# yoyololicon/pytorch-NMF

Hardware: AMD Instinct MI355X
Metric: MU GFLOP/s (algorithmic 8*N*C*R per iteration), dense NMF 4096x65536 rank-128 beta=1; MU iterations/s alongside (higher is better)
Workload: dtype f16; 1 GPU; NMF 4096x65536 rank=128 beta=1 (BASELINE configs[1]); preset=cfg1, rows=4096, cols_per_gpu=65536, rank=128, precision=f16, parallelism=single GPU, nsplit_h=16, nsplit_w=1, block_rows_h=256, block_rows_w=256, launch=eager launches

## Files before the change

include/nmfmu.h:

```cpp
#ifndef NMFMU_H_
#define NMFMU_H_

#include <stddef.h>
#include <stdint.h>

#ifdef __cplusplus
extern "C" {
#endif

#define NMFMU_ABI_VERSION 10

#define NMFMU_OK 0
#define NMFMU_ERR_UNSUPPORTED (-2)
#define NMFMU_ERR_ARG (-3)
#define NMFMU_ERR_ALLOC (-4)

#define NMFMU_PREC_BF16 0
#define NMFMU_PREC_BF16X3 1
#define NMFMU_PREC_F16 2
#define NMFMU_PREC_F16X 3
#define NMFMU_PREC_F16R 4

#define NMFMU_BETA_KL 0
#define NMFMU_BETA_EUC 1
#define NMFMU_BETA_IS 2
#define NMFMU_BETA_GEN 3

#define NMFMU_STAGE_REG 0
#define NMFMU_STAGE_DMA 1
#define NMFMU_STAGE_DMA_NOP2 3
#define NMFMU_STAGE_DMA_LDSTR 4
#define NMFMU_STAGE_DMA_SPLIT 2

typedef struct nmfmu_factor {
  float* f;
  void* p1_hi;
  void* p1_lo;
  void* p2_hi;
  void* p2_lo;
  float* colsum;
  float* colsum_part;
  int32_t rows;
  int32_t rows_pad;
} nmfmu_factor;

typedef struct nmfmu_step {
  const void* xp;
  nmfmu_factor owner;
  nmfmu_factor panel;
  float* slab_num;
  float* slab_den;
  int32_t rank;
  int32_t r_pad;
  int32_t nsplit;
  int32_t precision;
  int32_t stage;
  int32_t block_rows;
  float beta;
  float gamma;
  float l1, l2;
  uint32_t* status;
  void* stamps;
} nmfmu_step;

int nmfmu_abi_version(void);
int nmfmu_abi_check(int compiled_against);
int nmfmu_pad_rows(int rows);
int nmfmu_pad_rank(int rank);
int nmfmu_beta_kind(float beta);
int nmfmu_supported(int r_pad, int precision);
int nmfmu_block_rows(int r_pad, int precision, float beta);
int nmfmu_choose_nsplit(int owner_rows_pad, int panel_rows_pad, int block_rows, int num_cu);
#define NMFMU_KERNEL_FUSED 0
#define NMFMU_KERNEL_PP 1
#define NMFMU_KERNEL_SP 2
int nmfmu_kernel_family(int r_pad, int precision, float beta);
int nmfmu_pp_lds_transpose_supported(int r_pad, int precision, float beta);
int nmfmu_choose_nsplit_for(int owner_rows_pad, int panel_rows_pad, int r_pad, int precision, float beta, int block_rows, int num_cu);
int nmfmu_step_block_rows(int owner_rows_pad, int panel_rows_pad, int r_pad, int precision, float beta, int num_cu);
size_t nmfmu_xp_bytes(int owner_rows_pad, int panel_rows_pad, int precision);
size_t nmfmu_image_bytes(int rows_pad, int r_pad);
size_t nmfmu_slab_bytes(int owner_rows_pad, int r_pad, int nsplit);
size_t nmfmu_colsum_part_bytes(int rows_pad, int r_pad);

// ... 314 lines not shown
```

pytorch-nmf_amd/csrc/nmfmu_capi.hip:

```cpp
#include <hip/hip_runtime.h>
#include <stdint.h>

#include <algorithm>
#include <cstdlib>
#include <new>
#include <vector>

#include "../../include/nmfmu.h"
#include "nmfmu_aux.h"
#include "nmfmu_fused.h"
#include "nmfmu_pp.h"
#include "nmfmu_sp.h"
#include "nmfmu_sp2.h"

#ifndef NMFMU_SP
#define NMFMU_SP 1
#endif
#ifndef NMFMU_SP2
#define NMFMU_SP2 1
#endif
#ifndef NMFMU_FUSE_APPLY_TWO_ACC
#define NMFMU_FUSE_APPLY_TWO_ACC 1
#endif

using namespace nmfmu;

namespace {

inline hipStream_t S(void* s) { return reinterpret_cast<hipStream_t>(s); }
inline bool is_f16(int precision) {
  return precision == NMFMU_PREC_F16 || precision == NMFMU_PREC_F16X || precision == NMFMU_PREC_F16R;
}
inline bool x_is_f32(int precision) { return precision == NMFMU_PREC_BF16X3 || precision == NMFMU_PREC_F16X; }

#ifdef NMFMU_DEBUG_HOOKS
static int env_int(const char* name, int dflt) {
  const char* v = std::getenv(name);
  return v && *v ? std::atoi(v) : dflt;
}
static void* g_pp_debug = nullptr;
#endif
#ifndef NMFMU_PP_F16R
#define NMFMU_PP_F16R 1
#endif
static bool pp_eligible(int r_pad, int precision, float beta) {
  return nmfmu_beta_kind(beta) == NMFMU_BETA_KL && r_pad <= 128 &&
         (precision == NMFMU_PREC_F16 || precision == NMFMU_PREC_BF16 || (NMFMU_PP_F16R && precision == NMFMU_PREC_F16R));
}
static bool pp_ldstr_eligible(int r_pad, int precision, float beta) {
  return pp_eligible(r_pad, precision, beta) && pp_trl_available(r_pad, is_f16(precision) ? kOpF16 : kOpBf16, kModeMU);
}
static bool sp_eligible(int r_pad, int precision, float beta) {
  return NMFMU_SP && nmfmu_beta_kind(beta) == NMFMU_BETA_KL && r_pad == 256 && precision == NMFMU_PREC_F16;
}
static bool sp2_eligible(int r_pad, int precision, float beta) {
  const int k = nmfmu_beta_kind(beta);
  return NMFMU_SP2 && (k == NMFMU_BETA_IS || k == NMFMU_BETA_GEN) && r_pad == 128 && precision == NMFMU_PREC_F16;
}
static int kernel_beta_kind(float beta) {
  if (beta == 0.5f) return kSqrt;
  if (beta == 1.5f) return kSqrt3;
  return nmfmu_beta_kind(beta);
}

struct GramRef {
  const float* gram;
  const void* hi;
  const void* lo;
  const float* scale;
};

int fused_dispatch(const nmfmu_step* st, int mode, float* loss_part, int M, int K, hipStream_t s,
                   const float* fuse_kl_den = nullptr, bool fuse_apply = false, const GramRef* gm = nullptr) {
  if (!st || !st->owner.p1_hi || !st->panel.p1_hi) return NMFMU_ERR_ARG;
  if (!st->xp && (mode == kModeMU || mode == kModeXB)) return NMFMU_ERR_ARG;
  if (st->owner.rows_pad % kRowPad || st->panel.rows_pad % kRowPad) return NMFMU_ERR_ARG;
  if (st->block_rows != 128 && st->block_rows != 256) return NMFMU_ERR_ARG;
  if (st->stage != NMFMU_STAGE_DMA && st->stage != NMFMU_STAGE_DMA_SPLIT && st->stage != NMFMU_STAGE_DMA_NOP2 &&
      st->stage != NMFMU_STAGE_DMA_LDSTR)
    return NMFMU_ERR_UNSUPPORTED;
  const bool ldstr = st->stage == NMFMU_STAGE_DMA_LDSTR && mode != kModeLoss;
  if (ldstr && (mode != kModeMU || st->block_rows != 256 || !pp_ldstr_eligible(st->r_pad, st->precision, st->beta)))
    return NMFMU_ERR_UNSUPPORTED;
  if (st->stage == NMFMU_STAGE_DMA_SPLIT && mode == kModeMU && !(st->precision == NMFMU_PREC_BF16X3)) {
    if (nmfmu_beta_kind(st->beta) != NMFMU_BETA_KL || st->block_rows != 128) return NMFMU_ERR_UNSUPPORTED;
    mode = kModeMU2;
  }
  if (st->r_pad != pad_rank(st->rank) || st->nsplit < 1) return NMFMU_ERR_ARG;
  const bool x3 = st->precision == NMFMU_PREC_BF16X3;
  if (x3 && (!st->owner.p1_lo || !st->panel.p1_lo)) return NMFMU_ERR_ARG;
  const int kind = nmfmu_beta_kind(st->beta);
  if (st->precision == NMFMU_PREC_F16R && kind == NMFMU_BETA_EUC) return NMFMU_ERR_UNSUPPORTED;
  FusedArgs a{};
  a.xp = st->xp;
  a.p1_hi = static_cast<const uint16_t*>(st->panel.p1_hi);
  a.p1_lo = static_cast<const uint16_t*>(st->panel.p1_lo);
  a.p2_hi = static_cast<const uint16_t*>(st->panel.p2_hi);
  a.p2_lo = static_cast<const uint16_t*>(st->panel.p2_lo);
  a.a1_hi = static_cast<const uint16_t*>(st->owner.p1_hi);
  a.a1_lo = static_cast<const uint16_t*>(st->owner.p1_lo);
  a.slab_num = st->slab_num;
  a.slab_den = st->slab_den;
  a.loss_part = loss_part;
  a.M = M;
  a.K = K;
  a.M_pad = st->owner.rows_pad;
  a.ktiles = st->panel.rows_pad / kBK;
  a.nsplit = st->nsplit;
  a.tiles_per_split = (a.ktiles + st->nsplit - 1) / st->nsplit;
  a.beta = st->beta;
  a.status = st->status;
  a.cs_owner = st->owner.colsum;
  a.cs_panel = st->panel.colsum;
  if (fuse_apply) {
    a.fuse_apply = 1;
    a.rank = st->rank;
    a.f = st->owner.f;
    a.kl_den = fuse_kl_den;
    a.o1_hi = static_cast<uint16_t*>(st->owner.p1_hi), a.o1_lo = static_cast<uint16_t*>(st->owner.p1_lo);
    a.o2_hi = static_cast<uint16_t*>(st->owner.p2_hi), a.o2_lo = static_cast<uint16_t*>(st->owner.p2_lo);
    a.colsum_part = st->owner.colsum_part;
    a.l1 = st->l1, a.l2 = st->l2, a.gamma = st->gamma;
  }
  if (mode == kModeMU2) {
    if (!a.slab_num || !a.p2_hi || fuse_apply) return NMFMU_ERR_ARG;
  } else if (mode == kModeXB) {
    if (kind != kEuc || x3 || st->block_rows != 128) return NMFMU_ERR_UNSUPPORTED;
    if (!a.p2_hi || (!fuse_apply && !a.slab_num)) return NMFMU_ERR_ARG;
    if (fuse_apply && (!gm || st->r_pad > 128)) return NMFMU_ERR_ARG;
    if (gm) {
      if (!gm->hi || !gm->lo || !gm->scale || (!fuse_apply && !a.slab_den)) return NMFMU_ERR_ARG;
      a.gram_hi = static_cast<const uint16_t*>(gm->hi), a.gram_lo = static_cast<const uint16_t*>(gm->lo);
      a.gram_scale = gm->scale;
    } else {
      a.slab_den = nullptr;
    }
  } else if (mode == kModeMU || mode == kModeDen) {
    if (!a.slab_num || !a.p2_hi || (x3 && !a.p2_lo)) return NMFMU_ERR_ARG;
    if (mode == kModeMU && kind != kKL && !a.slab_den) return NMFMU_ERR_ARG;
    if (mode == kModeDen && (kind != kGen || st->block_rows != 128)) return NMFMU_ERR_UNSUPPORTED;
  } else if (!loss_part) {
    return NMFMU_ERR_ARG;
  }
  const int grid = (st->owner.rows_pad / st->block_rows) * st->nsplit;
  if (st->block_rows == 256) {
    if (!st->xp || mode == kModeDen || !pp_eligible(st->r_pad, st->precision, st->beta)) return NMFMU_ERR_UNSUPPORTED;
    a.tiles_per_split = (a.tiles_per_split + 1) & ~1;
    a.debug = mode == kModeMU ? st->stamps : nullptr;
#ifdef NMFMU_DEBUG_HOOKS
    if (mode == kModeMU && g_pp_debug) a.debug = g_pp_debug;
#endif
    if (ldstr) a.o2_hi = nullptr;
    return launch_pp(st->r_pad, is_f16(st->precision) ? kOpF16 : kOpBf16, mode, a, grid, s, st->precision == NMFMU_PREC_F16R,
                      mode == kModeMU && loss_part != nullptr, ldstr);
  }
  if (mode == kModeMU && sp_eligible(st->r_pad, st->precision, st->beta)) {
    a.tiles_per_split = (a.tiles_per_split + 3) & ~3;
    a.debug = st->stamps;
#ifdef NMFMU_DEBUG_HOOKS
    if (g_pp_debug) a.debug = g_pp_debug;
#endif
    if (st->stage == NMFMU_STAGE_DMA_NOP2) a.o2_hi = nullptr;
    return launch_sp(st->r_pad, kOpF16, a, grid, s);
  }
  if (mode == kModeMU && sp2_eligible(st->r_pad, st->precision, st->beta)) {
    a.tiles_per_split = (a.tiles_per_split + 3) & ~3;
    return launch_sp2(st->r_pad, kernel_beta_kind(st->beta), a, grid, s);
  }
  const int kk = kernel_beta_kind(st->beta);
#ifdef NMFMU_DEBUG_HOOKS
  a.debug = mode == kModeXB ? g_pp_debug : nullptr;
#endif
  switch (st->r_pad) {
    case 32: return launch_fused_r32(kk, st->precision, mode, a, grid, s);
    case 64: return launch_fused_r64(kk, st->precision, mode, a, grid, s);
    case 128: return launch_fused_r128(kk, st->precision, mode, a, grid, s);
    case 256: return launch_fused_r256(kk, st->precision, mode, a, grid, s);
  }
  return NMFMU_ERR_UNSUPPORTED;
}

struct Timer {
  std::vector<hipEvent_t> ev;
};

}

extern "C" {

int nmfmu_abi_version(void) { return NMFMU_ABI_VERSION; }
int nmfmu_abi_check(int compiled_against) { return compiled_against == NMFMU_ABI_VERSION ? NMFMU_OK : NMFMU_ERR_ARG; }
int nmfmu_pad_rows(int rows) { return rows <= 0 ? NMFMU_ERR_ARG : pad_rows(rows); }
int nmfmu_pad_rank(int rank) {
  const int r = pad_rank(rank);
  return r < 0 ? NMFMU_ERR_UNSUPPORTED : r;
}
int nmfmu_beta_kind(float beta) {
  if (beta == 1.f) return NMFMU_BETA_KL;
  if (beta == 2.f) return NMFMU_BETA_EUC;
  if (beta == 0.f) return NMFMU_BETA_IS;
  return NMFMU_BETA_GEN;
}
int nmfmu_supported(int r_pad, int precision) {
  if (r_pad != 32 && r_pad != 64 && r_pad != 128 && r_pad != 256) return 0;
  if (precision == NMFMU_PREC_BF16) return 1;
// ... 127 lines not shown
                                      st->owner.colsum, S(stream))
             : nmfmu_mu_apply(st, nullptr, nullptr, 0, kl ? kl_den : nullptr, stream);
  }
  return e;
}

int nmfmu_colsum_nparts(const nmfmu_step* st) {
  if (!st || (st->block_rows != 128 && st->block_rows != 256)) return NMFMU_ERR_ARG;
  return st->nsplit == 1 ? st->owner.rows_pad / st->block_rows : st->owner.rows_pad / apply_stripe_rows(st->owner.rows_pad);
}

int nmfmu_pack_nparts(int rows_pad) { return rows_pad <= 0 ? NMFMU_ERR_ARG : rows_pad / apply_stripe_rows(rows_pad); }

int nmfmu_colsum_finalize(const nmfmu_factor* fac, int nparts, int r_pad, void* stream) {
  if (!fac || !fac->colsum || !fac->colsum_part || nparts <= 0) return NMFMU_ERR_ARG;
  return launch_colsum_finalize(fac->colsum_part, nparts, r_pad, fac->colsum, S(stream));
}

int nmfmu_slab_reduce(const nmfmu_step* st, float* num_out, float* den_out, void* stream) {
  if (!st || !num_out || !st->slab_num) return NMFMU_ERR_ARG;
  const int64_t plane = (int64_t)st->owner.rows_pad * st->r_pad;
  int e = launch_slab_reduce(st->slab_num, st->nsplit, plane, num_out, S(stream));
  if (e) return e;
  if (den_out) {
    if (!st->slab_den) return NMFMU_ERR_ARG;
    e = launch_slab_reduce(st->slab_den, st->nsplit, plane, den_out, S(stream));
  }
  return e;
}

static int apply_common(const nmfmu_step* st, const float* num, const float* den, int nslab, const float* kl_den,
                        int trainer, float ortho, float* grad, void* stream, int den_nslab = 0, int skip_colsum = 0) {
  if (!st || !st->owner.f) return NMFMU_ERR_ARG;
  const bool kl = nmfmu_beta_kind(st->beta) == NMFMU_BETA_KL;
  ApplyArgs a{};
  a.f = st->owner.f;
  a.num = num ? num : st->slab_num;
  a.den = num ? den : st->slab_den;
  a.nslab = num ? nslab : st->nsplit;
  a.kl_den = kl ? kl_den : nullptr;
  if (!a.num || a.nslab < 1) return NMFMU_ERR_ARG;
  a.den_nslab = den_nslab;
  a.skip_colsum = skip_colsum;
  if (kl ? !a.kl_den : !a.den) return NMFMU_ERR_ARG;
  a.p1_hi = st->owner.p1_hi, a.p1_lo = st->owner.p1_lo, a.p2_hi = st->owner.p2_hi, a.p2_lo = st->owner.p2_lo;
  a.colsum_part = st->owner.colsum_part, a.colsum = st->owner.colsum;
  a.rows = st->owner.rows, a.rank = st->rank, a.rows_pad = st->owner.rows_pad;
  a.l1 = st->l1, a.l2 = st->l2, a.gamma = st->gamma;
  a.trainer = trainer, a.ortho = ortho, a.grad = grad;
  a.f16 = is_f16(st->precision);
  a.status = st->status;
  if (!a.p1_hi || !a.p2_hi || !a.colsum || !a.colsum_part) return NMFMU_ERR_ARG;
  if (st->stage == NMFMU_STAGE_DMA_NOP2 && sp_eligible(st->r_pad, st->precision, st->beta)) a.p2_hi = a.p2_lo = nullptr;
  if (st->stage == NMFMU_STAGE_DMA_LDSTR) {
    if (st->block_rows != 256 || !pp_ldstr_eligible(st->r_pad, st->precision, st->beta)) return NMFMU_ERR_UNSUPPORTED;
    a.p2_hi = a.p2_lo = nullptr;
  }
  return launch_apply(st->r_pad, a, st->precision == NMFMU_PREC_BF16X3, false, S(stream));
}

int nmfmu_mu_apply(const nmfmu_step* st, const float* num, const float* den, int nslab, const float* kl_den,
                   void* stream) {
  return apply_common(st, num, den, nslab, kl_den, 0, 0.f, nullptr, stream);
}

int nmfmu_trainer_apply(const nmfmu_step* st, const float* num, const float* den, int nslab, const float* kl_den,
                        float ortho, float* grad, void* stream) {
  if (!(ortho >= 0.f)) return NMFMU_ERR_ARG;
  return apply_common(st, num, den, nslab, kl_den, 1, ortho, grad, stream);
}

int nmfmu_xb_supported(int r_pad, int precision, float beta) {
  if (nmfmu_beta_kind(beta) != NMFMU_BETA_EUC) return 0;
  if (r_pad != 32 && r_pad != 64 && r_pad != 128 && r_pad != 256) return 0;
  if (precision == NMFMU_PREC_F16X) return r_pad <= 128;
  return precision == NMFMU_PREC_BF16 || precision == NMFMU_PREC_F16;
}

int nmfmu_xb_partial(const nmfmu_step* st, void* stream) {
  if (!st) return NMFMU_ERR_ARG;
  if (!nmfmu_xb_supported(st->r_pad, st->precision, st->beta)) return NMFMU_ERR_UNSUPPORTED;
  return fused_dispatch(st, kModeXB, nullptr, st->owner.rows, st->panel.rows, S(stream));
}

int nmfmu_xb_step(const nmfmu_step* st, const void* g_hi, const void* g_lo, const float* g_scale, int phase, void* stream) {
  if (!st || !g_hi || !g_lo || !g_scale || phase < 0 || phase > 2) return NMFMU_ERR_ARG;
  if (!nmfmu_xb_supported(st->r_pad, st->precision, st->beta)) return NMFMU_ERR_UNSUPPORTED;
  const bool fuse = st->nsplit == 1 && st->owner.f && st->owner.p2_hi && st->owner.colsum && st->owner.colsum_part &&
                    st->r_pad <= 128;
  if (!fuse && !st->slab_den) return NMFMU_ERR_ARG;
  const GramRef gm{nullptr, g_hi, g_lo, g_scale};
  int e = 0;
  if (phase != 2) {
    e = fused_dispatch(st, kModeXB, nullptr, st->owner.rows, st->panel.rows, S(stream), nullptr, fuse, &gm);
    if (e) return e;
  }
  if (phase != 1 && !fuse)
    e = apply_common(st, nullptr, nullptr, 0, nullptr, 0, 0.f, nullptr, stream, 1, 1);
  return e;
}

int nmfmu_mu_step_allreduce(const nmfmu_step* st, nmfmu_comm* comm, float* xbuf, void* stream) {
  if (!st || !comm || !xbuf) return NMFMU_ERR_ARG;
  const bool kl = nmfmu_beta_kind(st->beta) == NMFMU_BETA_KL;
  const size_t plane = (size_t)st->owner.rows_pad * st->r_pad;
  const size_t tail = kl ? (size_t)st->r_pad : plane;
  if (kl && !st->panel.colsum) return NMFMU_ERR_ARG;
// ... 228 lines not shown
```

pytorch-nmf_amd/torchnmf_amd/_capi.py:

```python
from __future__ import annotations

import ctypes as C
import os
from typing import Optional

LIB_NAME = 'libnmfmu.so'
LIB_PATH = os.environ.get('NMFMU_LIB') or os.path.join(os.path.dirname(os.path.abspath(__file__)), LIB_NAME)

OK = 0
ERR_UNSUPPORTED = -2
ERR_ARG = -3
ERR_ALLOC = -4
PREC_BF16, PREC_BF16X3, PREC_F16, PREC_F16X, PREC_F16R = 0, 1, 2, 3, 4
STAGE_REG, STAGE_DMA, STAGE_DMA_SPLIT = 0, 1, 2
STAGE_DMA_NOP2 = 3
STAGE_DMA_LDSTR = 4
BETA_KL, BETA_EUC, BETA_IS, BETA_GEN = 0, 1, 2, 3
KERNEL_FUSED, KERNEL_PP, KERNEL_SP = 0, 1, 2

PRECISIONS = {'bf16': PREC_BF16, 'bf16x3': PREC_BF16X3, 'f16': PREC_F16, 'f16x': PREC_F16X, 'f16r': PREC_F16R}


class NmfmuError(RuntimeError):
    pass


class Factor(C.Structure):
    _fields_ = [('f', C.c_void_p), ('p1_hi', C.c_void_p), ('p1_lo', C.c_void_p), ('p2_hi', C.c_void_p),
                ('p2_lo', C.c_void_p), ('colsum', C.c_void_p), ('colsum_part', C.c_void_p), ('rows', C.c_int32),
                ('rows_pad', C.c_int32)]


class Step(C.Structure):
    _fields_ = [('xp', C.c_void_p), ('owner', Factor), ('panel', Factor), ('slab_num', C.c_void_p),
                ('slab_den', C.c_void_p), ('rank', C.c_int32), ('r_pad', C.c_int32), ('nsplit', C.c_int32),
                ('precision', C.c_int32), ('stage', C.c_int32), ('block_rows', C.c_int32), ('beta', C.c_float), ('gamma', C.c_float),
                ('l1', C.c_float), ('l2', C.c_float), ('status', C.c_void_p), ('stamps', C.c_void_p)]


class GemmDesc(C.Structure):
    _fields_ = [('a_hi', C.c_void_p), ('a_lo', C.c_void_p), ('b_hi', C.c_void_p), ('b_lo', C.c_void_p),
                ('m_pad', C.c_int32), ('n_pad', C.c_int32), ('k_pad', C.c_int32), ('precision', C.c_int32),
                ('beta', C.c_float), ('x', C.c_void_p), ('gn_hi', C.c_void_p), ('gn_lo', C.c_void_p),
                ('gp_hi', C.c_void_p), ('gp_lo', C.c_void_p), ('out', C.c_void_p), ('m_valid', C.c_int32),
                ('n_valid', C.c_int32), ('ops', C.c_int32), ('t_batch', C.c_int32), ('t_rank', C.c_int32),
                ('t_taps', C.c_int32), ('t_lh', C.c_int32), ('tile_rows', C.c_int32), ('n_ld', C.c_int32), ('k_len', C.c_int32), ('k_split', C.c_int32),
                ('tail_rows', C.c_int32), ('rag_c0', C.c_int32), ('rag_channels', C.c_int32),
                ('win_nd', C.c_int32), ('win_lh', C.c_int32 * 3), ('win_taps', C.c_int32 * 3), ('win_channels', C.c_int32),
                ('win_pitch', C.c_int32), ('win_fold', C.c_int32), ('t_koff', C.c_void_p), ('stage_mode', C.c_int32)]


ABI_VERSION = 10
EPI_RATIO, EPI_F32, EPI_LOSS, EPI_FOLD = 0, 1, 2, 3
OPS_PLANES, OPS_B_HU, OPS_B_HUT, OPS_A_HU, OPS_A_WIN = 0, 1, 2, 3, 4

SIGNATURES = {
    'nmfmu_abi_version': (C.c_int, []),
    'nmfmu_abi_check': (C.c_int, [C.c_int]),
    'nmfmu_pad_rows': (C.c_int, [C.c_int]),
    'nmfmu_pad_rank': (C.c_int, [C.c_int]),
    'nmfmu_beta_kind': (C.c_int, [C.c_float]),
    'nmfmu_supported': (C.c_int, [C.c_int, C.c_int]),
    'nmfmu_block_rows': (C.c_int, [C.c_int, C.c_int, C.c_float]),
    'nmfmu_step_block_rows': (C.c_int, [C.c_int, C.c_int, C.c_int, C.c_int, C.c_float, C.c_int]),
    'nmfmu_choose_nsplit': (C.c_int, [C.c_int, C.c_int, C.c_int, C.c_int]),
    'nmfmu_kernel_family': (C.c_int, [C.c_int, C.c_int, C.c_float]),
    'nmfmu_pp_lds_transpose_supported': (C.c_int, [C.c_int, C.c_int, C.c_float]),
    'nmfmu_choose_nsplit_for': (C.c_int, [C.c_int, C.c_int, C.c_int, C.c_int, C.c_float, C.c_int, C.c_int]),
    'nmfmu_xp_bytes': (C.c_size_t, [C.c_int, C.c_int, C.c_int]),
# ... 238 lines not shown
```

pytorch-nmf_amd/torchnmf_amd/engine.py:

```python
from __future__ import annotations

import ctypes as C
import os
from typing import Optional

import torch

from . import _capi


def _ptr(t: Optional[torch.Tensor]) -> Optional[int]:
    return None if t is None else t.data_ptr()


class HipBackend:

    name = 'hip'

    def __init__(self):
        self.lib = _capi.load()
        if not torch.cuda.is_available():
            raise _capi.NmfmuError('torchnmf_amd needs a ROCm device (MI355X); none is visible and there is no '
                                   'CPU fallback')

# ... 389 lines not shown
            return None
        in_range, exact = cls.f16_stats(V, W, H, be) if dims_ok else (False, False)
        level = 2 if (in_range and exact) else (1 if in_range else 0)
        if level == 1 and not (hasattr(_capi, 'PREC_F16X') and be.supported(r_pad, _capi.PREC_F16X)
                               and os.environ.get('TORCHNMF_AMD_AUTO_F16X', '1') != '0'):
            level = 0
        if group is not None:
            import torch.distributed as dist
            flag = torch.tensor([level], dtype=torch.int32, device=V.device)
            dist.all_reduce(flag, op=dist.ReduceOp.MIN, group=group)
            level = int(flag.item())
            if level == 1 and not (hasattr(_capi, 'PREC_F16X') and be.supported(r_pad, _capi.PREC_F16X)):
                level = 0
        return {2: 'f16', 1: 'f16x', 0: None}[level]

    @classmethod
    def auto_mode(cls, V, W, H, r_pad, be, beta, group=None) -> Optional[str]:
        mode = cls.auto_single_plane(V, W, H, r_pad, be, group)
        if (mode == 'f16x' and float(beta) != 2.0 and hasattr(_capi, 'PREC_F16R') and be.supported(r_pad, _capi.PREC_F16R)
                and os.environ.get('TORCHNMF_AMD_AUTO_F16R', '1') != '0'):
            mode = 'f16r'
        return mode

    def __init__(self, V, W, H, beta, l1=0.0, l2=0.0, precision='auto', stage=None, group=None, backend=None,
                 update_W=True, update_H=True, block_rows=None, allow_f16=False, ar_overlap=None, allow_gram=False,
                 ar_direct=None):
        self.be = backend if backend is not None else DEFAULT_BACKEND_FACTORY()
        self.group = group
        self.beta = float(beta)
        self.kl = self.beta == 1.0
        N, Cc = V.shape
        R = W.shape[1]
        assert W.shape == (Cc, R) and H.shape == (N, R)
        if V.stride(1) != 1 or V.dtype != torch.float32:
            V = V.float().contiguous()
        self.rank = R
        self.r_pad = self.be.pad_rank(R)
        if precision in (None, 'auto'):
            precision = self.auto_mode(V, W, H, self.r_pad, self.be, self.beta, group) if allow_f16 else None
            if precision is None:
                if not self.be.supported(self.r_pad, _capi.PREC_BF16X3):
                    raise NotImplementedError(
                        f"precision='auto' found no mode for rank {R} that meets the 1e-4 parity bar on the fused kernels "
                        f"(fp16 operands -- 'f16', or 'f16x' with an fp32 target -- need both dimensions >= {self.F16_MIN_DIM} "
                        f"and data within fp16's range; split bf16 stops at rank 128); pass precision='bf16' (factors "
                        f"~1e-3), 'f16' or 'f16x' explicitly")
                precision = 'bf16x3'
        if precision not in _capi.PRECISIONS:
            raise ValueError(f"precision must be one of {sorted(_capi.PRECISIONS)} or 'auto', got {precision!r}")
        self.precision_name = precision
        self.precision = _capi.PRECISIONS[precision]
        if not self.be.supported(self.r_pad, self.precision):
            raise NotImplementedError(f'precision {precision!r} is not available for rank {R} (padded {self.r_pad})')
        if stage is None:
            nop2 = (hasattr(self.be, 'kernel_family') and hasattr(_capi, 'STAGE_DMA_NOP2') and float(beta) == 1.0
                    and self.r_pad == 256 and self.be.kernel_family(self.r_pad, self.precision, float(beta)) == _capi.KERNEL_SP
                    and os.environ.get('TORCHNMF_AMD_NO_P2', '1') != '0')
            stage = _capi.STAGE_DMA_NOP2 if nop2 else _capi.STAGE_DMA
            if (group is None and update_W and block_rows in (None, 256) and hasattr(self.be, 'pp_lds_transpose_supported')
                    and self.be.pp_lds_transpose_supported(self.r_pad, self.precision, float(beta))
                    and self.be.block_rows(self.r_pad, self.precision, float(beta)) == 256):
                stage = _capi.STAGE_DMA_LDSTR
        self.gram_path = (allow_gram and self.beta == 2.0 and group is None and block_rows in (None, 128)
                          and hasattr(self.be, 'xb_supported') and self.be.xb_supported(self.r_pad, self.precision, self.beta)
                          and os.environ.get('TORCHNMF_AMD_BETA2_GRAM', '1') != '0')
        gamma = mu_gamma(self.beta)
        dev = V.device

        self.fW = FactorBuf(W, self.r_pad, self.precision, self.be)
        self.fH = FactorBuf(H, self.r_pad, self.precision, self.be)
        self.flags = torch.tensor([0, 0x7f800000], dtype=torch.int32, device=dev)
        self.status = torch.zeros(1, dtype=torch.int32, device=dev)
        n_pad, c_pad = self.fH.rows_pad, self.fW.rows_pad
        def tile_rows(m_pad, k_pad):
            if block_rows is not None:
                return block_rows
            if hasattr(self.be, 'step_block_rows'):
                return self.be.step_block_rows(m_pad, k_pad, self.r_pad, self.precision, self.beta, dev)
            return self.be.block_rows(self.r_pad, self.precision, self.beta)
        br = tile_rows(n_pad, c_pad)
        self.block_rows = br
        xp_h = self.be.pack_x(V, False, self.precision, br, n_pad, c_pad, self.flags)
        ns_h = self._nsplit(n_pad, c_pad, br, dev)
        need_den = False if self.kl else ('one' if self.gram_path else True)
        self.step_h = StepBuf(xp_h, self.fH, self.fW, R, self.r_pad, ns_h, self.precision, stage, br, self.beta, gamma,
                              l1, l2, need_den=need_den, status=self.status)
        self.step_w = None
        if update_W:
            brw = tile_rows(c_pad, n_pad)
            xp_w = self.be.pack_x(V, True, self.precision, brw, c_pad, n_pad, None)
            ns_w = self._nsplit(c_pad, n_pad, brw, dev)
            self.step_w = StepBuf(xp_w, self.fW, self.fH, R, self.r_pad, ns_w, self.precision, stage, brw, self.beta,
                                  gamma, l1, l2, need_den=need_den, status=self.status)
        self.gm = self.be.gram_alloc(self.r_pad, dev) if self.gram_path else None
        self.timer: Optional[KernelTimer] = None
        self.refresh_images()
        self.loss_part = torch.empty(max((n_pad // br) * ns_h, 1), dtype=torch.float32, device=dev)
        self.loss_out = torch.zeros(1, dtype=torch.float64, device=dev)
        self._riding = None
        self._riding_pending = False
        if (group is None and self.kl and self.step_w is not None and update_H and hasattr(self.be, 'riding_supported')
                and os.environ.get('TORCHNMF_AMD_RIDING_LOSS', '1') != '0' and V.dtype == torch.float32 and V.stride(1) == 1
                and self.be.riding_supported(self.step_w)):
            self._riding = {'V': V, 'bufs': None}
        if group is not None:
            tail = self.r_pad if self.kl else self.step_h.plane
            self.xbuf = torch.empty(self.step_h.plane + tail, dtype=torch.float32, device=dev)
            explicit_direct = bool(ar_direct)
            if ar_direct is None:
                ar_direct = os.environ.get('TORCHNMF_AMD_COMM', 'torch') == 'c'
            self._comm = None
            if ar_direct and hasattr(self.be, 'comm_init'):
                self._comm = self.be.comm_init(group, dev)
                ar_overlap = False
            elif explicit_direct:
                raise _capi.NmfmuError("allreduce='direct' needs the library's own RCCL communicator (nmfmu_comm_*), which "
                                       f"the {getattr(self.be, 'name', type(self.be).__name__)} backend does not provide")
            st = self.step_h
            nblk = st.owner.rows_pad // 256
            frac = float(os.environ.get('TORCHNMF_AMD_AR_SPLIT', '0.5'))
            r0 = min(max(int(frac * nblk + 1e-9), 1), max(nblk - 1, 1)) * 256
            self._h_rows = None
            if ar_overlap is None:
                ar_overlap = os.environ.get('TORCHNMF_AMD_AR_OVERLAP', '0') != '0'
            if (ar_overlap and nblk >= 2 and st.owner.rows > r0
                    and hasattr(self.be, 'xp_rows')):
                k_pad = st.panel.rows_pad
                parts = [(0, r0), (r0, st.owner.rows_pad - r0)]
                ns = [StepRows.nsplit_for(st, n, self.be, k_pad, dev) for _, n in parts]
                need = sum(k * n * self.r_pad for k, (_, n) in zip(ns, parts))
                big_n = torch.empty(max(need, st.nsplit * st.plane), dtype=torch.float32, device=dev)
                big_d = None if st.slab_den is None else torch.empty_like(big_n)
                st.slab_num, st.slab_den = big_n[:st.nsplit * st.plane], (None if big_d is None else big_d[:st.nsplit * st.plane])
                st.struct.slab_num, st.struct.slab_den = _ptr(st.slab_num), _ptr(st.slab_den)
                self._h_rows, off = [], 0
                for k, (a0, n) in zip(ns, parts):
                    cnt = k * n * self.r_pad
                    self._h_rows.append(StepRows(st, a0, n, self.be, k_pad, k, big_n[off:off + cnt],
                                                 None if big_d is None else big_d[off:off + cnt]))
                    off += cnt

    def repack_target(self, V):
        st = self.step_h
        assert tuple(V.shape) == (st.owner.rows, st.panel.rows), 'repack_target: shape differs from the bound target'
        if V.stride(1) != 1 or V.dtype != torch.float32:
            V = V.float().contiguous()
# ... 177 lines not shown
```

Measured before the change: 936,500 GFLOP/s.

## Add software-pipelined rank-128 f16 KL MU kernel with LDS-transpose and DMA staging

Result: faster. 975,700 GFLOP/s (median of 6 runs) (+4.2%).

```diff
diff --git a/include/nmfmu.h b/include/nmfmu.h
--- a/include/nmfmu.h
+++ b/include/nmfmu.h
@@ -30,6 +30,7 @@
 #define NMFMU_STAGE_DMA 1
 #define NMFMU_STAGE_DMA_NOP2 3
 #define NMFMU_STAGE_DMA_LDSTR 4
+#define NMFMU_STAGE_DMA_SP128 5
 #define NMFMU_STAGE_DMA_SPLIT 2
 
 typedef struct nmfmu_factor {
diff --git a/pytorch-nmf_amd/csrc/nmfmu_capi.hip b/pytorch-nmf_amd/csrc/nmfmu_capi.hip
--- a/pytorch-nmf_amd/csrc/nmfmu_capi.hip
+++ b/pytorch-nmf_amd/csrc/nmfmu_capi.hip
@@ -12,6 +12,7 @@
 #include "nmfmu_pp.h"
 #include "nmfmu_sp.h"
 #include "nmfmu_sp2.h"
+#include "nmfmu_sp128.h"
 
 #ifndef NMFMU_SP
 #define NMFMU_SP 1
@@ -49,6 +50,9 @@
 }
 static bool pp_ldstr_eligible(int r_pad, int precision, float beta) {
   return pp_eligible(r_pad, precision, beta) && pp_trl_available(r_pad, is_f16(precision) ? kOpF16 : kOpBf16, kModeMU);
+}
+static bool sp128_eligible(int r_pad, int precision, float beta) {
+  return pp_ldstr_eligible(r_pad, precision, beta) && precision == NMFMU_PREC_F16 && sp128_available(r_pad, kOpF16, kModeMU);
 }
 static bool sp_eligible(int r_pad, int precision, float beta) {
   return NMFMU_SP && nmfmu_beta_kind(beta) == NMFMU_BETA_KL && r_pad == 256 && precision == NMFMU_PREC_F16;
@@ -77,11 +81,13 @@
   if (st->owner.rows_pad % kRowPad || st->panel.rows_pad % kRowPad) return NMFMU_ERR_ARG;
   if (st->block_rows != 128 && st->block_rows != 256) return NMFMU_ERR_ARG;
   if (st->stage != NMFMU_STAGE_DMA && st->stage != NMFMU_STAGE_DMA_SPLIT && st->stage != NMFMU_STAGE_DMA_NOP2 &&
-      st->stage != NMFMU_STAGE_DMA_LDSTR)
+      st->stage != NMFMU_STAGE_DMA_LDSTR && st->stage != NMFMU_STAGE_DMA_SP128)
     return NMFMU_ERR_UNSUPPORTED;
-  const bool ldstr = st->stage == NMFMU_STAGE_DMA_LDSTR && mode != kModeLoss;
+  const bool sp128 = st->stage == NMFMU_STAGE_DMA_SP128;
+  const bool ldstr = (st->stage == NMFMU_STAGE_DMA_LDSTR || sp128) && mode != kModeLoss;
   if (ldstr && (mode != kModeMU || st->block_rows != 256 || !pp_ldstr_eligible(st->r_pad, st->precision, st->beta)))
     return NMFMU_ERR_UNSUPPORTED;
+  if (sp128 && !sp128_eligible(st->r_pad, st->precision, st->beta)) return NMFMU_ERR_UNSUPPORTED;
   if (st->stage == NMFMU_STAGE_DMA_SPLIT && mode == kModeMU && !(st->precision == NMFMU_PREC_BF16X3)) {
     if (nmfmu_beta_kind(st->beta) != NMFMU_BETA_KL || st->block_rows != 128) return NMFMU_ERR_UNSUPPORTED;
     mode = kModeMU2;
@@ -151,6 +157,10 @@
     if (mode == kModeMU && g_pp_debug) a.debug = g_pp_debug;
 #endif
     if (ldstr) a.o2_hi = nullptr;
+    if (sp128 && mode == kModeMU && !loss_part) {
+      a.tiles_per_split = (a.tiles_per_split + 3) & ~3;
+      return launch_sp128(st->r_pad, kOpF16, a, grid, s);
+    }
     return launch_pp(st->r_pad, is_f16(st->precision) ? kOpF16 : kOpBf16, mode, a, grid, s, st->precision == NMFMU_PREC_F16R,
                       mode == kModeMU && loss_part != nullptr, ldstr);
   }
@@ -384,7 +394,7 @@
   a.status = st->status;
   if (!a.p1_hi || !a.p2_hi || !a.colsum || !a.colsum_part) return NMFMU_ERR_ARG;
   if (st->stage == NMFMU_STAGE_DMA_NOP2 && sp_eligible(st->r_pad, st->precision, st->beta)) a.p2_hi = a.p2_lo = nullptr;
-  if (st->stage == NMFMU_STAGE_DMA_LDSTR) {
+  if (st->stage == NMFMU_STAGE_DMA_LDSTR || st->stage == NMFMU_STAGE_DMA_SP128) {
     if (st->block_rows != 256 || !pp_ldstr_eligible(st->r_pad, st->precision, st->beta)) return NMFMU_ERR_UNSUPPORTED;
     a.p2_hi = a.p2_lo = nullptr;
   }
diff --git a/pytorch-nmf_amd/csrc/nmfmu_inst_sp128.hip b/pytorch-nmf_amd/csrc/nmfmu_inst_sp128.hip
--- /dev/null
+++ b/pytorch-nmf_amd/csrc/nmfmu_inst_sp128.hip
@@ -0,0 +1,12 @@
+#include "nmfmu_sp128.h"
+
+namespace nmfmu {
+
+bool sp128_available(int r_pad, int opt, int mode) { return r_pad == 128 && opt == kOpF16 && mode == kModeMU; }
+
+int launch_sp128(int r_pad, int opt, const FusedArgs& a, int grid, hipStream_t s) {
+  if (r_pad == 128 && opt == kOpF16) return launch_sp128_one<kOpF16>(a, grid, s);
+  return -2;
+}
+
+}
diff --git a/pytorch-nmf_amd/csrc/nmfmu_sp128.h b/pytorch-nmf_amd/csrc/nmfmu_sp128.h
--- /dev/null
+++ b/pytorch-nmf_amd/csrc/nmfmu_sp128.h
@@ -0,0 +1,484 @@
+#pragma once
+#include "nmfmu_sp.h"
+
+namespace nmfmu {
+
+template <int OPT>
+struct SP128Cfg {
+  static constexpr int R_PAD = 128;
+  static constexpr int BM = 256, WAVES = 4, THREADS = 256;
+  static constexpr int KS = R_PAD / 16, RT = R_PAD / 32, ROWB = 2 * R_PAD, IMG = kBK * ROWB;
+  static constexpr int NSLOT = 4, PF = 4;
+  static constexpr int N1 = 2 * KS, N2 = 4 * RT;
+  static constexpr int NPW = IMG / 1024 / WAVES;
+  static constexpr int XTILE = BM * kBK * 2;
+  static constexpr int GOPS = 10;
+  static constexpr int NEL = 16 * GOPS;
+  static constexpr int LDS_MAIN = NSLOT * IMG;
+  static constexpr int LDS_EPI = 2 * WAVES * 32 * R_PAD * 4;
+  static constexpr int LDS_BYTES = LDS_MAIN > LDS_EPI ? LDS_MAIN : LDS_EPI;
+  static_assert(OPT == kOpF16, "fp16 operands");
+  static_assert(N1 == 16 && N2 == 16 && NPW == 4 && NSLOT * IMG <= 65536, "schedule tables below; every LDS offset an immediate");
+};
+
+template <int OPT>
+__global__ void __launch_bounds__(256, 1) sp128_kernel(const FusedArgs a) {
+  using C = SP128Cfg<OPT>;
+  constexpr int R_PAD = C::R_PAD, KS = C::KS, RT = C::RT, ROWB = C::ROWB, IMG = C::IMG, PF = C::PF, N1 = C::N1, N2 = C::N2;
+  using u32x2 = __attribute__((ext_vector_type(2))) uint32_t;
+  extern __shared__ __attribute__((aligned(16))) char smem[];
+
+  const int tid = threadIdx.x;
+  const int lane = tid & 63;
+  const int wave = __builtin_amdgcn_readfirstlane(tid >> 6);
+  const int j = lane & 31;
+  const int hl = lane >> 5;
+  const int mb = blockIdx.x / a.nsplit;
+  const int ks = blockIdx.x - mb * a.nsplit;
+  const int t0 = ks * a.tiles_per_split;
+  const int t1 = min(t0 + a.tiles_per_split, a.ktiles);
+  const int nt = t1 - t0;
+
+  asm volatile("s_setreg_imm32_b32 hwreg(HW_REG_MODE, 23, 1), 1");
+  auto stamp = [&](int slot) {
+    unsigned long long* dbg = reinterpret_cast<unsigned long long*>(a.debug);
+    if (!dbg || wave != 0) return;
+    const unsigned long long c = __builtin_amdgcn_s_memtime();
+    const unsigned long long r = __builtin_amdgcn_s_memrealtime();
+    if (lane == 0) {
+      if (blockIdx.x == 0) {
+        dbg[slot * 4 + 0] = c;
+        dbg[slot * 4 + 1] = r;
+        dbg[slot * 4 + 2] = (unsigned long long)(nt > 0 ? nt : 0);
+      }
+      dbg[64 + 5 * blockIdx.x + slot] = r;
+      if (slot == 2)
+        dbg[64 + 5 * blockIdx.x + 4] = ((unsigned long long)__builtin_amdgcn_s_getreg(20 | (31 << 11)) << 32) |
+                                       (unsigned long long)__builtin_amdgcn_s_getreg(4 | (31 << 11));
+    }
+  };
+  stamp(2);
+
+  f32x16 acc[2][RT];
+#pragma unroll
+  for (int og = 0; og < 2; ++og)
+#pragma unroll
+    for (int rt = 0; rt < RT; ++rt)
+#pragma unroll
+      for (int e = 0; e < 16; ++e) acc[og][rt][e] = 0.f;
+  static_for<2 * RT>([&](auto rc) {
+    f32x16& r = acc[decltype(rc)::value / RT][decltype(rc)::value % RT];
+    asm volatile("" : "+a"(r));
+  });
+
+  if (nt > 0) {
+    const unsigned lds_base =
+        __builtin_amdgcn_readfirstlane((unsigned)(size_t)(__attribute__((address_space(3))) char*)smem);
+    const unsigned ldsw = lds_base + (unsigned)wave * (unsigned)(C::NPW * 1024);
+    const char* xsrc = reinterpret_cast<const char*>(a.xp) + ((size_t)mb * a.ktiles + t0) * (size_t)C::XTILE + (size_t)wave * 8192;
+    const char* p1src = reinterpret_cast<const char*>(a.p1_hi) + (size_t)t0 * IMG;
+    asm volatile("" : "+s"(xsrc), "+s"(p1src));
+    const unsigned lane16 = (unsigned)lane * 16u;
+    const unsigned dv = (unsigned)wave * (unsigned)(C::NPW * 1024) + lane16;
+    auto clampt = [&](int t) { return t < nt ? t : nt - 1; };
+    auto panel_src = [&](int t) {
+      const char* p = p1src + (size_t)clampt(t) * IMG;
+      asm volatile("" : "+s"(p));
+      return p;
+    };
+    auto x_src = [&](int t, int og) {
+      const char* p = xsrc + (size_t)clampt(t) * (size_t)C::XTILE + (size_t)og * 4096;
+      asm volatile("" : "+s"(p));
+      return p;
+    };
+
+    u32x4 q[2][KS];
+#pragma unroll
+    for (int og = 0; og < 2; ++og) {
+      const int m0 = mb * C::BM + (2 * wave + og) * 32 + j;
+      const int sw = P1Swz<R_PAD>::of(m0) << 4;
+      const char* row = reinterpret_cast<const char*>(a.a1_hi) + (size_t)m0 * ROWB;
+#pragma unroll
+      for (int kk = 0; kk < KS; ++kk) q[og][kk] = ld16(row + ((kk * 32 + hl * 16) ^ sw));
+    }
+
+    const int row0 = 32 * ((j >> 2) & 1) + (j & 3) + 4 * (j >> 3);
+    const int sw0 = P1Swz<R_PAD>::of(row0);
+    int ga[KS];
+#pragma unroll
+    for (int v = 0; v < KS; ++v) ga[v] = row0 * ROWB + (((2 * v + hl) ^ sw0) << 4);
+    const int grp = lane >> 4, s16 = lane & 15;
+    const int cslot = 2 * (grp & 1) + ((s16 & 3) >> 1), lr = (s16 >> 2) & 3;
+    int gb[4][RT];
+#pragma unroll
+    for (int c = 0; c < 4; ++c)
+#pragma unroll
+      for (int p = 0; p < RT; ++p)
+        gb[c][p] = (32 * (grp >> 1) + (s16 >> 2)) * ROWB + (((cslot ^ c) | ((lr ^ p) << 2)) << 4) + 8 * (s16 & 1);
+
+    f32x16 epsv;
+#pragma unroll
+    for (int e = 0; e < 16; ++e) epsv[e] = kEps;
+    asm volatile("" : "+v"(epsv));
+
+    f32x16 S[2][2][2];
+    u32x4 xb[2][2][4];
+    uint32_t gn[2][2][8];
+    u32x4 r128[PF];
+    u32x2 rlo[PF], rhi[PF];
+    float er[4];
+
+    auto dma_piece = [&](const char* src_tile, auto pc, auto slotc) {
+      constexpr int p = decltype(pc)::value, off = decltype(slotc)::value * IMG;
+      const unsigned vo = dv, lw = ldsw;
+      asm volatile("s_add_u32 m0, %2, %3\n\ts_nop 0\n\tglobal_load_lds_dwordx4 %0, %1 offset:%4"
+                   :
+                   : "v"(vo), "s"(src_tile), "s"(lw), "n"(off), "n"(p * 1024)
+                   : "memory", "m0", "scc");
+    };
+    auto load_x1 = [&](const char* src, u32x4(&x)[4], auto qc) {
+      constexpr int qi = decltype(qc)::value;
+      const unsigned l16 = lane16;
+      u32x4& dst = x[qi];
+      asm volatile("global_load_dwordx4 %0, %1, %2 offset:%3 nt" : "=&v"(dst) : "v"(l16), "s"(src), "n"(qi * 1024) : "memory");
+    };
+    auto wait_x = [&](auto cntc, u32x4(&x)[2][4]) {
+      asm volatile("s_waitcnt vmcnt(%8)"
+                   : "+v"(x[0][0]), "+v"(x[0][1]), "+v"(x[0][2]), "+v"(x[0][3]), "+v"(x[1][0]), "+v"(x[1][1]), "+v"(x[1][2]), "+v"(x[1][3])
+                   : "n"(decltype(cntc)::value)
+                   : "memory");
+    };
+    auto barrier = [&]() { asm volatile("s_barrier" ::: "memory"); };
+    auto ratio_op = [&](auto kc, auto sbc) {
+      constexpr int k = decltype(kc)::value, sb = decltype(sbc)::value, GO = C::GOPS;
+      constexpr int g = k / GO, pos = k % GO, og = g >> 3, tt = (g >> 2) & 1, d = 2 * (g & 3);
+      if constexpr (pos < 4) {
+        float& r = er[pos];
+        const float sv = S[sb][og][tt][2 * d + pos];
+        asm volatile("v_rcp_f32 %0, %1" : "=v"(r) : "v"(sv));
+      } else if constexpr (pos < 8) {
+        constexpr int p = pos - 4;
+        float& r = er[p];
+        const uint32_t w = xb[sb][og][2 * tt + (d >> 2)][(d & 3) + (p >> 1)];
+        if constexpr ((p & 1) == 0) asm volatile("v_fma_mix_f32 %0, %1, %0, 0 op_sel_hi:[1,0,0]" : "+v"(r) : "v"(w));
+        else asm volatile("v_fma_mix_f32 %0, %1, %0, 0 op_sel:[1,0,0] op_sel_hi:[1,0,0]" : "+v"(r) : "v"(w));
+      } else {
+        constexpr int h = pos - 8;
+        uint32_t& g2 = gn[og][tt][d + h];
+        const float e0 = er[2 * h], e1 = er[2 * h + 1];
+        asm volatile("v_cvt_pk_f16_f32 %0, %1, %2" : "=v"(g2) : "v"(e0), "v"(e1));
+      }
+    };
+    auto issue_g1 = [&](auto kc, auto slotc, auto rsc) {
+      constexpr int k = decltype(kc)::value, tt = k & 1, kk = k >> 1, rs = decltype(rsc)::value;
+      u32x4& dst = r128[rs];
+      const int ad = ga[kk];
+      asm volatile("ds_read_b128 %0, %1 offset:%2" : "=v"(dst) : "v"(ad), "n"(tt * 16 * ROWB + decltype(slotc)::value * IMG));
+    };
+    auto issue_g2 = [&](auto kc, auto slotc, auto rsc) {
+      constexpr int k = decltype(kc)::value, rt = k % RT, c4 = k / RT, tt = c4 >> 1, m2 = c4 & 1, rs = decltype(rsc)::value;
+      constexpr int o0 = (16 * tt + 8 * m2) * ROWB + decltype(slotc)::value * IMG;
+      u32x2 &dlo = rlo[rs], &dhi = rhi[rs];
+      const int a0 = gb[2 * m2][rt], a1 = gb[2 * m2 + 1][rt];
+      asm volatile("ds_read_b64_tr_b16 %0, %1 offset:%2" : "=v"(dlo) : "v"(a0), "n"(o0));
+      asm volatile("ds_read_b64_tr_b16 %0, %1 offset:%2" : "=v"(dhi) : "v"(a1), "n"(o0 + 4 * ROWB));
+    };
+    auto mfma_g1 = [&](auto kc, auto nbc, auto rsc, auto ogc) {
+      constexpr int k = decltype(kc)::value, tt = k & 1, kk = k >> 1, nb = decltype(nbc)::value, rs = decltype(rsc)::value;
+      constexpr int og = decltype(ogc)::value;
+      f32x16& sd = S[nb][og][tt];
+      const u32x4 pa = r128[rs], qo = q[og][kk];
+      const f32x16 seed = epsv;
+      if constexpr (kk == 0) asm volatile("v_mfma_f32_32x32x16_f16 %0, %1, %2, %3" : "=&v"(sd) : "v"(pa), "a"(qo), "v"(seed));
+      else asm volatile("v_mfma_f32_32x32x16_f16 %0, %1, %2, %0" : "+v"(sd) : "v"(pa), "a"(qo));
+    };
+    auto mfma_g2 = [&](auto kc, auto rsc, auto ogc) {
+      constexpr int k = decltype(kc)::value, rt = k % RT, c4 = k / RT, tt = c4 >> 1, m2 = c4 & 1, rs = decltype(rsc)::value;
+      constexpr int og = decltype(ogc)::value;
+      const u32x4 nh = {gn[og][tt][4 * m2], gn[og][tt][4 * m2 + 1], gn[og][tt][4 * m2 + 2], gn[og][tt][4 * m2 + 3]};
+      const u32x4 bh = {rlo[rs][0], rlo[rs][1], rhi[rs][0], rhi[rs][1]};
+      f32x16& ad = acc[og][rt];
+      asm volatile("v_mfma_f32_32x32x16_f16 %0, %1, %2, %0" : "+a"(ad) : "v"(nh), "v"(bh));
+    };
+    auto issue_entry = [&](auto nc, auto lastc) {
+      constexpr int n = decltype(nc)::value;
+      constexpr SPEnt e = sp_entry<N1, N2>(n, decltype(lastc)::value);
+      using RS = std::integral_constant<int, n % PF>;
+      if constexpr (e.g1) issue_g1(std::integral_constant<int, e.k>{}, std::integral_constant<int, (e.it + 1) & 3>{}, RS{});
+      else issue_g2(std::integral_constant<int, e.k>{}, std::integral_constant<int, e.it & 3>{}, RS{});
+    };
+    auto ratio_gap = [&](auto gapc, auto sbc) {
+      constexpr int gi = decltype(gapc)::value, per = C::NEL / 32;
+      static_assert(C::NEL % 32 == 0, "whole instructions per gap");
+      static_for<per>([&](auto cc) { ratio_op(std::integral_constant<int, gi * per + decltype(cc)::value>{}, sbc); });
+    };
+
+    auto group = [&](int i0, auto lastc) {
+      constexpr bool last = decltype(lastc)::value;
+      constexpr int LEN = sp_group_len<N1, N2>(last);
+      const char* dsrc = nullptr;
+      const char* xs0 = nullptr;
+      const char* xs1 = nullptr;
+      static_for<PF>([&](auto pc) { issue_entry(pc, lastc); });
+      static_for<LEN>([&](auto nc) {
+        constexpr int n = decltype(nc)::value;
+        constexpr SPEnt e = sp_entry<N1, N2>(n, last);
+        constexpr bool final_it = last && e.it == 3;
+        using RS = std::integral_constant<int, n % PF>;
+        using K = std::integral_constant<int, e.k>;
+        using SB = std::integral_constant<int, e.it & 1>;
+        using OG0 = std::integral_constant<int, 0>;
+        using OG1 = std::integral_constant<int, 1>;
+        if constexpr (final_it && e.k == 0)
+          static_for<C::NEL>([&](auto kc) { ratio_op(kc, SB{}); });
+        asm volatile("s_waitcnt lgkmcnt(%0)" ::"n"(sp_younger<N1, N2, PF>(n, last)));
+        if constexpr (e.g1) {
+          using NB = std::integral_constant<int, (e.it + 1) & 1>;
+          mfma_g1(K{}, NB{}, RS{}, OG0{});
+          if constexpr (e.k == 0) {
+            dsrc = panel_src(i0 + e.it + 3);
+            xs0 = x_src(i0 + e.it + 2, 0);
+            xs1 = x_src(i0 + e.it + 2, 1);
+          }
+          ratio_gap(std::integral_constant<int, 2 * e.k>{}, SB{});
+          mfma_g1(K{}, NB{}, RS{}, OG1{});
+          if constexpr (n + PF < LEN) issue_entry(std::integral_constant<int, n + PF>{}, lastc);
+          ratio_gap(std::integral_constant<int, 2 * e.k + 1>{}, SB{});
+          if constexpr (e.k == N1 - 1) {
+            asm volatile("s_waitcnt vmcnt(8)" ::: "memory");
+            barrier();
+          }
+        } else {
+          mfma_g2(K{}, RS{}, OG0{});
+          if constexpr (!final_it) {
+            if constexpr (e.k < C::NPW) dma_piece(dsrc, K{}, std::integral_constant<int, (e.it + 3) & 3>{});
+            if constexpr (e.k >= 8 && e.k < 12) load_x1(xs0, xb[e.it & 1][0], std::integral_constant<int, e.k - 8>{});
+            if constexpr (e.k >= 12) load_x1(xs1, xb[e.it & 1][1], std::integral_constant<int, e.k - 12>{});
+          }
+          mfma_g2(K{}, RS{}, OG1{});
+          if constexpr (n + PF < LEN) issue_entry(std::integral_constant<int, n + PF>{}, lastc);
+          if constexpr (!final_it && e.k == N2 - 1) {
+            wait_x(std::integral_constant<int, 12>{}, xb[(e.it + 1) & 1]);
+          }
+        }
+      });
+    };
+
+    {
+      static_for<3>([&](auto tc) {
+        const char* src = panel_src(decltype(tc)::value);
+        asm volatile("s_nop 4" ::: "memory");
+        static_for<C::NPW>([&](auto pc) { dma_piece(src, pc, tc); });
+      });
+      const char* x00 = x_src(0, 0);
+      const char* x01 = x_src(0, 1);
+      const char* x10 = x_src(1, 0);
+      const char* x11 = x_src(1, 1);
+      asm volatile("s_nop 4" ::: "memory");
+      static_for<4>([&](auto qc) { load_x1(x00, xb[0][0], qc); });
+      static_for<4>([&](auto qc) { load_x1(x01, xb[0][1], qc); });
+      static_for<4>([&](auto qc) { load_x1(x10, xb[1][0], qc); });
+      static_for<4>([&](auto qc) { load_x1(x11, xb[1][1], qc); });
+      wait_x(std::integral_constant<int, 0>{}, xb[0]);
+      wait_x(std::integral_constant<int, 0>{}, xb[1]);
+      static_for<2 * KS>([&](auto kc) {
+        u32x4& r = q[decltype(kc)::value / KS][decltype(kc)::value % KS];
+        asm volatile("" : "+a"(r));
+      });
+      barrier();
+      using Z = std::integral_constant<int, 0>;
+      static_for<PF>([&](auto pc) { issue_g1(pc, Z{}, pc); });
+      static_for<N1>([&](auto kc) {
+        constexpr int k = decltype(kc)::value;
+        constexpr int younger = (N1 - 1 - k) < (PF - 1) ? (N1 - 1 - k) : (PF - 1);
+        asm volatile("s_waitcnt lgkmcnt(%0)" ::"n"(younger));
+        mfma_g1(kc, Z{}, std::integral_constant<int, k % PF>{}, Z{});
+        mfma_g1(kc, Z{}, std::integral_constant<int, k % PF>{}, std::integral_constant<int, 1>{});
+        if constexpr (k + PF < N1) issue_g1(std::integral_constant<int, k + PF>{}, Z{}, std::integral_constant<int, k % PF>{});
+      });
+      asm volatile("s_nop 15\n\ts_nop 7" ::: "memory");
+    }
+    stamp(0);
+    int i0 = 0;
+    for (; i0 + 4 < nt; i0 += 4) group(i0, std::false_type{});
+    group(i0, std::true_type{});
+    stamp(1);
+    asm volatile("s_nop 15\n\ts_nop 15" ::: "memory");
+    wait_x(std::integral_constant<int, 0>{}, xb[0]);
+    wait_x(std::integral_constant<int, 0>{}, xb[1]);
+  }
+  __syncthreads();
+
+  int tid_e = tid;
+  asm volatile("" : "+v"(tid_e));
+  const int lane_e = tid_e & 63, j_e = lane_e & 31, hl_e = lane_e >> 5;
+  if (a.fuse_apply) {
+    constexpr int LDT = R_PAD;
+    constexpr int SP = R_PAD / 8;
+    constexpr int NCH = (32 * SP) / 64;
+    const int slot_e = lane_e % SP, rl0 = lane_e / SP;
+    float den8[8];
+#pragma unroll
+    for (int k = 0; k < 8; ++k) den8[k] = a.kl_den[slot_e * 8 + k];
+    const bool vec = (a.rank & 3) == 0;
+    bool clamped = false;
+    static_for<2 * RT>([&](auto rc) {
+      constexpr int og = decltype(rc)::value / RT, rt = decltype(rc)::value % RT;
+      float* tile = reinterpret_cast<float*>(smem) + (2 * wave + og) * (32 * LDT);
+#pragma unroll
+      for (int e = 0; e < 16; ++e) tile[((e & 3) + 8 * (e >> 2) + 4 * hl_e) * LDT + rt * 32 + j_e] = acc[og][rt][e];
+    });
+    __syncthreads();
+    const bool plain = a.l1 <= 0.f && a.l2 <= 0.f && a.gamma == 1.f && a.rank == R_PAD && mb * C::BM + C::BM <= a.M;
+    float csum8[2][8], rden8[8];
+#pragma unroll
+    for (int k = 0; k < 8; ++k) rden8[k] = 1.f / den8[k];
+#pragma unroll
+    for (int og = 0; og < 2; ++og) {
+      float* tile = reinterpret_cast<float*>(smem) + (2 * wave + og) * (32 * LDT);
+      const int mrow0 = mb * C::BM + (2 * wave + og) * 32;
+#pragma unroll
+      for (int k = 0; k < 8; ++k) csum8[og][k] = 0.f;
+      if (plain) {
+#pragma unroll 4
+        for (int i = 0; i < NCH; ++i) {
+          const int rl = i * (64 / SP) + rl0, row = mrow0 + rl, r0 = slot_e * 8;
+          float* trow = tile + rl * LDT + r0;
+          float* frow = a.f + (size_t)row * R_PAD + r0;
+          float fv[8], nm[8];
+          *reinterpret_cast<float4*>(fv) = *reinterpret_cast<const float4*>(frow);
+          *reinterpret_cast<float4*>(fv + 4) = *reinterpret_cast<const float4*>(frow + 4);
+          *reinterpret_cast<float4*>(nm) = *reinterpret_cast<const float4*>(trow);
+          *reinterpret_cast<float4*>(nm + 4) = *reinterpret_cast<const float4*>(trow + 4);
+#pragma unroll
+          for (int k = 0; k < 8; ++k) {
+            const float mult = (fmaxf(nm[k], 0.f) + kEps) * rden8[k];
+            csum8[og][k] = __builtin_fmaf(fv[k], mult, csum8[og][k]);
+            fv[k] *= mult;
+            clamped |= fv[k] > 65504.f;
+          }
+          *reinterpret_cast<float4*>(frow) = *reinterpret_cast<const float4*>(fv);
+          *reinterpret_cast<float4*>(frow + 4) = *reinterpret_cast<const float4*>(fv + 4);
+          if (a.o2_hi) {
+            *reinterpret_cast<float4*>(trow) = *reinterpret_cast<const float4*>(fv);
+            *reinterpret_cast<float4*>(trow + 4) = *reinterpret_cast<const float4*>(fv + 4);
+          }
+          u32x4 hi;
+#pragma unroll
+          for (int qq = 0; qq < 4; ++qq) hi[qq] = pack_op<OPT>(fv[2 * qq], fv[2 * qq + 1]);
+          *reinterpret_cast<u32x4*>(reinterpret_cast<char*>(a.o1_hi) + p1_offset(row, r0, R_PAD)) = hi;
+        }
+      } else {
+#pragma unroll 2
+        for (int i = 0; i < NCH; ++i) {
+          const int rl = i * (64 / SP) + rl0, row = mrow0 + rl, r0 = slot_e * 8;
+          float* trow = tile + rl * LDT + r0;
+          float* frow = a.f + (size_t)row * a.rank + r0;
+          float fv[8], nm[8];
+          *reinterpret_cast<float4*>(nm) = *reinterpret_cast<const float4*>(trow);
+          *reinterpret_cast<float4*>(nm + 4) = *reinterpret_cast<const float4*>(trow + 4);
+#pragma unroll
+          for (int h = 0; h < 2; ++h) {
+            const bool in = row < a.M && r0 + 4 * h < a.rank;
+            if (in && vec) {
+              *reinterpret_cast<float4*>(fv + 4 * h) = *reinterpret_cast<const float4*>(frow + 4 * h);
+            } else {
+#pragma unroll
+              for (int k = 0; k < 4; ++k) fv[4 * h + k] = (in && r0 + 4 * h + k < a.rank) ? frow[4 * h + k] : 0.f;
+            }
+          }
+#pragma unroll
+          for (int k = 0; k < 8; ++k) {
+            const float neg = fmaxf(nm[k], 0.f) + kEps;
+            float pos = den8[k];
+            if (a.l1 > 0.f) pos += a.l1;
+            if (a.l2 > 0.f) pos += a.l2 * fv[k];
+            float mult = neg / pos;
+            if (a.gamma != 1.f) mult = mu_pow(mult, a.gamma);
+            fv[k] = (row < a.M && r0 + k < a.rank) ? fv[k] * mult : 0.f;
+            csum8[og][k] += fv[k];
+            clamped |= fv[k] > 65504.f;
+          }
+#pragma unroll
+          for (int h = 0; h < 2; ++h) {
+            const bool in = row < a.M && r0 + 4 * h < a.rank;
+            if (in && vec) {
+              *reinterpret_cast<float4*>(frow + 4 * h) = *reinterpret_cast<const float4*>(fv + 4 * h);
+            } else if (in) {
+#pragma unroll
+              for (int k = 0; k < 4; ++k)
+                if (r0 + 4 * h + k < a.rank) frow[4 * h + k] = fv[4 * h + k];
+            }
+          }
+          *reinterpret_cast<float4*>(trow) = *reinterpret_cast<const float4*>(fv);
+          *reinterpret_cast<float4*>(trow + 4) = *reinterpret_cast<const float4*>(fv + 4);
+          u32x4 hi;
+#pragma unroll
+          for (int qq = 0; qq < 4; ++qq) hi[qq] = pack_op<OPT>(fv[2 * qq], fv[2 * qq + 1]);
+          *reinterpret_cast<u32x4*>(reinterpret_cast<char*>(a.o1_hi) + p1_offset(row, r0, R_PAD)) = hi;
+        }
+      }
+    }
+    if (a.status && __any(clamped) && lane_e == 0) atomicOr(a.status, 1u);
+    if (a.o2_hi) {
+      __syncthreads();
+#pragma unroll
+      for (int og = 0; og < 2; ++og) {
+        const float* tile = reinterpret_cast<const float*>(smem) + (2 * wave + og) * (32 * LDT);
+        const int mrow0 = mb * C::BM + (2 * wave + og) * 32;
+#pragma unroll
+        for (int ii = 0; ii < R_PAD / 64; ++ii) {
+          const int r = ii * 64 + lane_e;
+#pragma unroll
+          for (int g = 0; g < 4; ++g) {
+            const float* src = tile + (g * 8) * LDT + r;
+            u32x4 hi;
+#pragma unroll
+            for (int qq = 0; qq < 4; ++qq) hi[qq] = pack_op<OPT>(src[(2 * qq) * LDT], src[(2 * qq + 1) * LDT]);
+            *reinterpret_cast<u32x4*>(reinterpret_cast<char*>(a.o2_hi) + p2_offset(mrow0 + g * 8, r, R_PAD)) = hi;
+          }
+        }
+      }
+    }
+    __syncthreads();
+    float* red = reinterpret_cast<float*>(smem);
+#pragma unroll
+    for (int og = 0; og < 2; ++og)
+#pragma unroll
+      for (int k = 0; k < 8; ++k) {
+        float tot = csum8[og][k];
+        tot += __shfl_xor(tot, 32, 64);
+        tot += __shfl_xor(tot, 16, 64);
+        if (lane_e < SP) red[(2 * wave + og) * R_PAD + slot_e * 8 + k] = tot;
+      }
+    __syncthreads();
+    for (int r = tid_e; r < R_PAD; r += C::THREADS) {
+      float tot = (red[r] + red[R_PAD + r]) + (red[2 * R_PAD + r] + red[3 * R_PAD + r]);
+      tot += (red[4 * R_PAD + r] + red[5 * R_PAD + r]) + (red[6 * R_PAD + r] + red[7 * R_PAD + r]);
+      a.colsum_part[(size_t)mb * R_PAD + r] = tot;
+    }
+  } else {
+    static_for<2 * RT>([&](auto rc) {
+      constexpr int og = decltype(rc)::value / RT, rt = decltype(rc)::value % RT;
+      const size_t slab = ((size_t)ks * a.M_pad + (size_t)(mb * C::BM + (2 * wave + og) * 32)) * R_PAD;
+#pragma unroll
+      for (int e = 0; e < 16; ++e) {
+        const int row = (e & 3) + 8 * (e >> 2) + 4 * hl_e;
+        a.slab_num[slab + (size_t)row * R_PAD + rt * 32 + j_e] = acc[og][rt][e];
+      }
+    });
+  }
+  if (a.debug) asm volatile("s_waitcnt vmcnt(0)" ::: "memory");
+  stamp(3);
+}
+
+template <int OPT>
+int launch_sp128_one(const FusedArgs& a, int grid, hipStream_t s) {
+  using C = SP128Cfg<OPT>;
+  return launch_with_dynamic_lds<sp128_kernel<OPT>, C::THREADS, C::LDS_BYTES>(dim3(grid), s, a);
+}
+
+int launch_sp128(int r_pad, int opt, const FusedArgs& a, int grid, hipStream_t s);
+bool sp128_available(int r_pad, int opt, int mode);
+
+}
diff --git a/pytorch-nmf_amd/torchnmf_amd/_capi.py b/pytorch-nmf_amd/torchnmf_amd/_capi.py
--- a/pytorch-nmf_amd/torchnmf_amd/_capi.py
+++ b/pytorch-nmf_amd/torchnmf_amd/_capi.py
@@ -15,6 +15,7 @@
 STAGE_REG, STAGE_DMA, STAGE_DMA_SPLIT = 0, 1, 2
 STAGE_DMA_NOP2 = 3
 STAGE_DMA_LDSTR = 4
+STAGE_DMA_SP128 = 5
 BETA_KL, BETA_EUC, BETA_IS, BETA_GEN = 0, 1, 2, 3
 KERNEL_FUSED, KERNEL_PP, KERNEL_SP = 0, 1, 2
 
diff --git a/pytorch-nmf_amd/torchnmf_amd/engine.py b/pytorch-nmf_amd/torchnmf_amd/engine.py
--- a/pytorch-nmf_amd/torchnmf_amd/engine.py
+++ b/pytorch-nmf_amd/torchnmf_amd/engine.py
@@ -465,6 +465,7 @@
         self.precision = _capi.PRECISIONS[precision]
         if not self.be.supported(self.r_pad, self.precision):
             raise NotImplementedError(f'precision {precision!r} is not available for rank {R} (padded {self.r_pad})')
+        sp128_auto = False
         if stage is None:
             nop2 = (hasattr(self.be, 'kernel_family') and hasattr(_capi, 'STAGE_DMA_NOP2') and float(beta) == 1.0
                     and self.r_pad == 256 and self.be.kernel_family(self.r_pad, self.precision, float(beta)) == _capi.KERNEL_SP
@@ -474,6 +475,7 @@
                     and self.be.pp_lds_transpose_supported(self.r_pad, self.precision, float(beta))
                     and self.be.block_rows(self.r_pad, self.precision, float(beta)) == 256):
                 stage = _capi.STAGE_DMA_LDSTR
+                sp128_auto = self.precision == _capi.PREC_F16 and os.environ.get('TORCHNMF_AMD_SP128', '1') != '0'
         self.gram_path = (allow_gram and self.beta == 2.0 and group is None and block_rows in (None, 128)
                           and hasattr(self.be, 'xb_supported') and self.be.xb_supported(self.r_pad, self.precision, self.beta)
                           and os.environ.get('TORCHNMF_AMD_BETA2_GRAM', '1') != '0')
@@ -505,6 +507,13 @@
             ns_w = self._nsplit(c_pad, n_pad, brw, dev)
             self.step_w = StepBuf(xp_w, self.fW, self.fH, R, self.r_pad, ns_w, self.precision, stage, brw, self.beta,
                                   gamma, l1, l2, need_den=need_den, status=self.status)
+        if sp128_auto and dev.type == 'cuda':
+            ncu = torch.cuda.get_device_properties(dev).multi_processor_count
+            steps = (self.step_h, self.step_w)
+            if all(st.block_rows == 256 and (st.owner.rows_pad // 256) * st.nsplit >= ncu
+                   and (st.panel.rows_pad // 64) % (4 * st.nsplit) == 0 for st in steps):
+                for st in steps:
+                    st.struct.stage = _capi.STAGE_DMA_SP128
         self.gm = self.be.gram_alloc(self.r_pad, dev) if self.gram_path else None
         self.timer: Optional[KernelTimer] = None
         self.refresh_images()
```
